# rasmusab/bayes.js

Hardware: AMD Instinct MI355X
Metric: posterior draws/sec (= param-updates/sec) (higher is better)
Workload: dtype f64

## Files before the change

bayes.js_amd/csrc/amwg_kernel.h:

```cpp
#pragma once
#if !defined(__HIPCC_RTC__)
#include <hip/hip_runtime.h>
#endif

#include "amwg_div.h"
#include "amwg_ld.h"
#include "amwg_philox.h"
#include "amwg_types.h"

namespace amwg {

struct LdsLayout {
  uint32_t data, state, pls, cnt, tot, cc, adapt, pl, idx, perm, total, stride, logpls, bc, xw;
};
__host__ __device__ inline LdsLayout lds_layout(size_t data_bytes, int P, int CPB, int max_top, int n_named, bool multi = false) {
  LdsLayout L;
  uint32_t o = 0;
  L.stride = (uint32_t)P | 1u;
  L.data = o;  o += (uint32_t)((data_bytes + 15) & ~(size_t)15);
  L.state = o; o += L.stride * CPB * 8;
  L.pls = o;   o += L.stride * CPB * 8;
  L.cnt = o;   o += L.stride * CPB * 8;
  L.tot = o;   o += (L.stride * CPB * 4 + 15) & ~15u;
  L.cc = o;    o += (uint32_t)P * sizeof(CompConst);
  L.adapt = o; o += ((uint32_t)P + 7) & ~7u;
  L.pl = o;    o += (uint32_t)n_named * 20u;
  o = (o + 15) & ~15u;
  L.idx = o;   o += (max_top > 1) ? (((uint32_t)max_top * CPB * (max_top > kByteTop ? 2u : 1u) + 15) & ~15u) : 0;
  L.perm = o;  o += (n_named > kPackedNamed) ? (((uint32_t)n_named * CPB * 2u + 15) & ~15u) : 0;
  L.logpls = o; o += multi ? L.stride * CPB * 8 : 0;
  L.bc = o;     o += multi ? ((L.stride * CPB * 4 + 15) & ~15u) : 0;
  L.xw = o;     o += multi ? 2u * 16u * 8u : 0;
  L.total = (o + 15) & ~15u;
  return L;
}

template <class Model, bool FAST, int G, int U = Model::kUnroll>
__device__ __forceinline__ double pass_over_data(const typename Model::Pass &ps, int n_obs, int sub, double acc) {
  const int n_full = n_obs / G, rem = n_obs % G;
  int k = 0;
  for (; k + U <= n_full; k += U) {
    double t[U];
#pragma unroll
    for (int u = 0; u < U; ++u) t[u] = Model::template term<FAST>(ps, (k + u) * G + sub);
#pragma unroll
    for (int u = 0; u < U; ++u) acc += t[u];
  }
  for (; k < n_full; ++k) acc += Model::template term<FAST>(ps, k * G + sub);
  if (sub < rem) acc += Model::template term<FAST>(ps, n_full * G + sub);
  return acc;
}

struct CrossWave {
  double *buf;
  int parity;
};

template <class...> using void_of = void;

template <class M, class = void> struct BinaryOf { static constexpr bool value = true; };
template <class M> struct BinaryOf<M, void_of<decltype(M::kHasBinary)>> { static constexpr bool value = M::kHasBinary; };

template <class M, class = void> struct TracksState { static constexpr bool value = false; };
template <class M> struct TracksState<M, void_of<decltype(M::kTracksState)>> { static constexpr bool value = M::kTracksState; };

template <class M, class = void> struct LaneReuseOf { static constexpr bool value = false; };
template <class M> struct LaneReuseOf<M, void_of<decltype(M::kLaneReuse)>> { static constexpr bool value = M::kLaneReuse; };

template <class M, class = void> struct CertifiedOf { static constexpr bool value = false; static constexpr int lanes = 0; };
template <class M> struct CertifiedOf<M, void_of<decltype(M::kCertified)>> { static constexpr bool value = M::kCertified; static constexpr int lanes = M::kCertifiedLanes; };
template <class M, int G, class = void> struct CertifiedAt { static constexpr bool value = false; };
template <class M, int G> struct CertifiedAt<M, G, void_of<decltype(M::kCertified)>> { static constexpr bool value = M::kCertified && M::kCertifiedLanes == G; };

template <class M, class = void> struct CertNeedsRows { static constexpr bool value = false; };
template <class M> struct CertNeedsRows<M, void_of<decltype(M::kCertifiedNeedsRows)>> { static constexpr bool value = M::kCertifiedNeedsRows; };

template <class M, class = void> struct RefOrderOf { static constexpr bool value = false; };
template <class M> struct RefOrderOf<M, void_of<decltype(M::kReferenceOrder)>> { static constexpr bool value = M::kReferenceOrder; };

template <class M, class = void> struct OwnPassOf { static constexpr bool value = false; };
template <class M> struct OwnPassOf<M, void_of<decltype(M::kOwnPass)>> { static constexpr bool value = M::kOwnPass; };

struct NoCache {};
template <class M, class = void> struct CacheOf { using type = NoCache; static __device__ __forceinline__ type init() { return type{}; } };
template <class M> struct CacheOf<M, void_of<typename M::Cache>> { using type = typename M::Cache; static __device__ __forceinline__ type init() { return M::cache_init(); } };

template <int OFF, bool EXACT = false>
__device__ __forceinline__ double xor_partner(double v) {
#if defined(__HIP_DEVICE_COMPILE__)
  int lo = (int)(uint32_t)f64_bits(v), hi = (int)(uint32_t)(f64_bits(v) >> 32);
  if constexpr (OFF == 1) {
    lo = __builtin_amdgcn_mov_dpp(lo, 0xB1, 0xF, 0xF, true); hi = __builtin_amdgcn_mov_dpp(hi, 0xB1, 0xF, 0xF, true);
  } else if constexpr (OFF == 2) {
    lo = __builtin_amdgcn_mov_dpp(lo, 0x4E, 0xF, 0xF, true); hi = __builtin_amdgcn_mov_dpp(hi, 0x4E, 0xF, 0xF, true);
  } else if constexpr (OFF == 4) {
    lo = __builtin_amdgcn_mov_dpp(lo, 0x141, 0xF, 0xF, true); hi = __builtin_amdgcn_mov_dpp(hi, 0x141, 0xF, 0xF, true);
    if constexpr (EXACT) {
      lo = __builtin_amdgcn_mov_dpp(lo, 0x1B, 0xF, 0xF, true); hi = __builtin_amdgcn_mov_dpp(hi, 0x1B, 0xF, 0xF, true);
    }
  } else if constexpr (OFF == 8) {
    lo = __builtin_amdgcn_mov_dpp(lo, 0x140, 0xF, 0xF, true); hi = __builtin_amdgcn_mov_dpp(hi, 0x140, 0xF, 0xF, true);
    if constexpr (EXACT) {
      lo = __builtin_amdgcn_mov_dpp(lo, 0x141, 0xF, 0xF, true); hi = __builtin_amdgcn_mov_dpp(hi, 0x141, 0xF, 0xF, true);
    }
  } else if constexpr (OFF == 16) {
    lo = __builtin_amdgcn_ds_swizzle(lo, 0x401F); hi = __builtin_amdgcn_ds_swizzle(hi, 0x401F);
  } else {
    return __shfl_xor(v, OFF, 64);
  }
  return bits_f64(((uint64_t)(uint32_t)hi << 32) | (uint64_t)(uint32_t)lo);
#else
  return v;
#endif
}
template <int OFF, bool EXACT = false>
__device__ __forceinline__ double xor_sum(double acc) {
#if defined(__HIP_DEVICE_COMPILE__)
  if constexpr (OFF == 16 || OFF == 32) {
    const uint32_t lo = (uint32_t)f64_bits(acc), hi = (uint32_t)(f64_bits(acc) >> 32);
    if constexpr (OFF == 32) {
      const auto l = __builtin_amdgcn_permlane32_swap(lo, lo, false, false), h = __builtin_amdgcn_permlane32_swap(hi, hi, false, false);
      return bits_f64(((uint64_t)h[0] << 32) | (uint64_t)l[0]) + bits_f64(((uint64_t)h[1] << 32) | (uint64_t)l[1]);
    } else {
      const auto l = __builtin_amdgcn_permlane16_swap(lo, lo, false, false), h = __builtin_amdgcn_permlane16_swap(hi, hi, false, false);
      return bits_f64(((uint64_t)h[0] << 32) | (uint64_t)l[0]) + bits_f64(((uint64_t)h[1] << 32) | (uint64_t)l[1]);
    }
  } else {
    return acc + xor_partner<OFF, EXACT>(acc);
  }
#else
  return acc;
#endif
}
template <int OFF, int LIMIT>
__device__ __forceinline__ double butterfly(double acc) {
  if constexpr (OFF < LIMIT) { acc = xor_sum<OFF>(acc); return butterfly<OFF * 2, LIMIT>(acc); }
  else return acc;
}

#ifndef AMWG_STEPPER_PRIORITY
#define AMWG_STEPPER_PRIORITY 2
#endif
constexpr int kStepperPriority = AMWG_STEPPER_PRIORITY;
__device__ __forceinline__ void wave_priority(int p) {
#if defined(__HIP_DEVICE_COMPILE__)
  if (kStepperPriority > 0) { if (p == 0) __builtin_amdgcn_s_setprio(0); else __builtin_amdgcn_s_setprio(kStepperPriority); }
#endif
}

__device__ __forceinline__ int fresh_uniform(int v) {
#if defined(__HIP_DEVICE_COMPILE__)
#if !defined(AMWG_X_NOFRESH)
  v = __builtin_amdgcn_readfirstlane(v);
  asm volatile("" : "+s"(v));
#endif
#endif
  return v;
}

template <class Model, int G, int U = 8>
__device__ __forceinline__ double log_post(const StateView &S, const StepArgs &a0, const unsigned char *smem, int sub, CrossWave &xw,
// ... 285 lines not shown
#else
  return v;
#endif
}

constexpr int kErrReplicasNeedOneWave = 1, kErrLaunchTooLong = 2, kErrMirrorOutOfSync = 4, kErrSweepNeedsOrderInRegisters = 8, kErrNoKernelBody = 16;
__device__ __forceinline__ void device_error(const StepArgs &a, int code) {
#if defined(__HIP_DEVICE_COMPILE__)
  if (threadIdx.x == 0) (void)atomicOr(a.ch.error, code);
#endif
}
template <class M, class = void> struct MirrorCheckOf { static constexpr bool value = false; };
template <class M> struct MirrorCheckOf<M, void_of<decltype(M::kMirrorCheck)>> { static constexpr bool value = M::kMirrorCheck; };

template <class Model, int G, int BT = 256, bool GL = false, bool SW = false, bool CT = false>
__device__ __forceinline__ void step_body(const StepArgs &a, unsigned char *smem) {
  constexpr int kPassU = SW ? (CertNeedsRows<Model>::value ? 2 : 4) : (BT >= 1024 ? 4 : 8);
  const int tid = threadIdx.x, nt = blockDim.x;
  constexpr bool kMulti = G > 64;
  if (!kMulti && a.cpb > 0 && nt != 64) { device_error(a, kErrReplicasNeedOneWave); return; }
  if (a.n_steps > 65535) { device_error(a, kErrLaunchTooLong); return; }
  const int CPB = kMulti ? G / 64 : ((a.cpb > 0 && a.cpb < nt / G) ? a.cpb : nt / G);
  const int c_raw = kMulti ? tid / 64 : tid / G;
  const int c_in = c_raw < CPB ? c_raw : CPB - 1, sub = tid % G;
  const int P = a.pl.P;
  const int n_named = a.pl.n_params;
  const LdsLayout L = lds_layout(DataBytesOf<Model, GL>::get(a.d, G, nt), P, CPB, a.pl.max_top, n_named, kMulti);

  const unsigned char *data_lds = smem + L.data;
  double *Sblk = reinterpret_cast<double *>(smem + L.state);
  CompConst *cc = reinterpret_cast<CompConst *>(smem + L.cc);
  uint8_t *adapt = smem + L.adapt;
  int32_t *pl_base = reinterpret_cast<int32_t *>(smem + L.pl), *pl_len = pl_base + n_named, *pl_top = pl_len + n_named, *pl_multidim = pl_top + n_named, *pl_inner = pl_multidim + n_named;
  const bool wide_idx = a.pl.max_top > kByteTop, wide_perm = n_named > kPackedNamed;
  const IndexColumn idx{smem + L.idx + (wide_idx ? 2 * c_in : c_in), CPB, wide_idx};
  const IndexColumn pcol{smem + L.perm + 2 * c_in, CPB, true};
  double *SDme = reinterpret_cast<double *>(smem + L.pls) + (size_t)c_in * L.stride;
  int2 *CNTme = reinterpret_cast<int2 *>(smem + L.cnt) + (size_t)c_in * L.stride;
  uint32_t *TOTme = reinterpret_cast<uint32_t *>(smem + L.tot) + (size_t)c_in * L.stride;
  double *LOGPLSme = reinterpret_cast<double *>(smem + L.logpls) + (size_t)c_in * L.stride;
  int32_t *BCme = reinterpret_cast<int32_t *>(smem + L.bc) + (size_t)c_in * L.stride;
  CrossWave xw{reinterpret_cast<double *>(smem + L.xw), 0};
  typename CacheOf<Model>::type cache = CacheOf<Model>::init();

  Model::stage(smem + L.data, a.d, tid, nt, G);
  for (int p = tid; p < P; p += nt) { cc[p] = a.cc[p]; adapt[p] = a.is_adapting[p]; }
  for (int i = tid; i < 4 * n_named; i += nt) pl_base[i] = a.pl.tab[i];
  for (int i = tid; i < n_named; i += nt) pl_inner[i] = a.pl.tab[n_named + i] / a.pl.tab[2 * n_named + i];

  const int64_t chain_raw = kMulti ? (int64_t)blockIdx.x : (int64_t)blockIdx.x * CPB + c_in;
  const bool live = chain_raw < a.C;
  const int64_t cl = live ? chain_raw : a.C - 1;
  const bool writer = live && sub == 0;
  const bool counter = sub == 0 && c_raw < CPB;
  const int64_t C = a.C;

  double *Sme = Sblk + (size_t)c_in * L.stride;
  for (int p = 0; p < P; ++p) {
    Sme[p] = a.ch.state[p * C + cl];
    SDme[p] = exp_v8(a.ch.prop_log_scale[p * C + cl]);
    CNTme[p] = make_int2(a.ch.acceptance_count[p * C + cl], a.ch.iterations_since_adaption[p * C + cl]);
    TOTme[p] = 0u;
    if constexpr (kMulti) { LOGPLSme[p] = a.ch.prop_log_scale[p * C + cl]; BCme[p] = a.ch.batch_count[p * C + cl]; }
  }
  const StateView S{Sme};
  uint64_t perm = wide_perm ? 0ull : a.ch.perm[cl];
  if (wide_perm)
    for (int k = 0; k < n_named; ++k) pcol.set(k, (int)a.ch.perm16[(int64_t)k * C + cl]);
  typename RngOf<Model, G, GL, SW>::type rng;
  if constexpr (GL) rng.init(a.seed, a.chain_offset + (uint64_t)cl, a.ch.rng_n[cl], tid, reinterpret_cast<double *>(smem + L.data + Model::gl_lds_bytes(a.d.pad, 0)) + (size_t)(tid >> 6) * 256);
  else if constexpr (SW) rng.init(a.seed, a.chain_offset + (uint64_t)cl, a.ch.rng_n[cl], tid, reinterpret_cast<double *>(smem + L.data + Model::window_offset(a.d, nt / 64)) + (size_t)(tid >> 6) * 256);
  else rng.init(a.seed, a.chain_offset + (uint64_t)cl, a.ch.rng_n[cl], tid);
  double lp_curr = a.ch.lp_curr[cl];
  __syncthreads();
  constexpr bool kCert = CT && CertifiedAt<Model, G>::value && !GL && (SW == CertNeedsRows<Model>::value);
  static_assert(kCert == CT, "a certified kernel is instantiated for a model that has no certified value at this lane count");
  constexpr bool kRefOrder = kCert && G > 1 && RefOrderOf<Model>::value;
  auto expression = [&]() -> double {
    if constexpr (kRefOrder) return Model::template reference_order<G>(cache, S, a.mc, a.d, data_lds, sub);
    else if constexpr (!GL) return log_post<Model, G, kPassU>(S, a, data_lds, sub, xw, cache);
    else return 0.0;
  };
  if constexpr (!GL) { if (a.init_lp) lp_curr = expression(); }
  double lpA = lp_curr, epsA = 0.0;
  bool lp_exact = true;
  if constexpr (kCert) { if (!a.init_lp) { epsA = a.ch.lp_eps[cl]; lp_exact = epsA == 0.0; } }
  (void)lpA; (void)epsA; (void)lp_exact;
#if defined(AMWG_AUDIT)
  constexpr bool kAudit = kCert;
#else
  constexpr bool kAudit = false;
#endif
  [[maybe_unused]] double audE = 0.0, aud_max_v = 0.0, aud_max_d = 0.0;
  [[maybe_unused]] uint32_t aud_n = 0u, aud_bad = 0u;
  [[maybe_unused]] auto audit_bin = [&](int which, double ratio) {
#if defined(AMWG_AUDIT)
    if (writer) {
      int b = 0;
      if (ratio > 0.0) { b = (int)((f64_bits(ratio) >> 52) & 0x7ffu) - 1023 + 40; b = b < 1 ? 1 : (b > 63 ? 63 : b); }
      if (!(ratio == ratio)) b = 63;
      (void)atomicAdd(cold_args()->ch.audit_hist + which * 64 + b, 1ull);
    }
#endif
  };
  [[maybe_unused]] auto audit_adversarial_u = [&](double ex, double eta, double u, int parity) -> double {
    if (!(eta < 0x1p-8) || !(ex > 0x1p-900) || !(ex < kInf)) return u;
    const double below = ex * (1.0 - 1.5 * eta), above = ex * (1.0 + 1.5 * eta);
    const double v = ((parity & 1) && above < 1.0) ? above : below;
    return (v > 0.0 && v < 1.0) ? v : u;
  };
  [[maybe_unused]] auto audit_value = [&](double A, double eps, double E) {
    if (eps == eps && eps < kInf && eps > 0.0 && E == E && __builtin_fabs(E) < kInf) {
      const double r = __builtin_fabs(A - E) / eps;
      aud_max_v = (r > aud_max_v || !(r == r)) ? r : aud_max_v;
      audit_bin(0, r);
    }
  };
  [[maybe_unused]] auto audit_difference = [&](double dA, double eta0, double dE, int verdict, double u) {
    if (eta0 == eta0 && eta0 < kInf && eta0 > 0.0 && dE == dE && __builtin_fabs(dE) < kInf) {
      const double r = __builtin_fabs(dA - dE) / eta0;
      aud_max_d = (r > aud_max_d || !(r == r)) ? r : aud_max_d;
      audit_bin(1, r);
    }
    const bool exact_acc = exp_v8(dE) > u;
    ++aud_n;
    if ((verdict > 0 && !exact_acc) || (verdict < 0 && exact_acc)) ++aud_bad;
  };
#if defined(AMWG_X_PHASES)
  uint64_t ph_acc[16];
#pragma unroll
  for (int q = 0; q < 16; ++q) ph_acc[q] = 0;
  uint64_t ph_last = __builtin_readcyclecounter();
#define AMWG_PHASE(i) do { const uint64_t ph_now = __builtin_readcyclecounter(); ph_acc[i] += ph_now - ph_last; ph_last = ph_now; } while (0)
#else
#define AMWG_PHASE(i) do { } while (0)
#endif
  auto set_state = [&](int comp, double v) {
    Sme[comp] = v;
    if constexpr (TracksState<Model>::value) Model::on_set(cache, comp, v, sub, a.d);
  };

  constexpr int D = Model::kDerived;
  const int PR = P + D;
  int64_t row = a.row0;
  int32_t next_rec = (int32_t)a.step0;
  const int P_stepped = a.pl.P_stepped;
  const bool recording = a.draws != nullptr;
  const int n_steps = a.n_steps;

  const int lane64 = tid & 63;
  int ord = lane64;
  (void)ord;
  if (SW && a.pl.max_top > 64) { device_error(a, kErrSweepNeedsOrderInRegisters); return; }
  const bool ord_in_regs = SW ? true : (G >= 64 && a.pl.max_top <= 64);
  constexpr bool kSweep = SW && !GL && LaneReuseOf<Model>::value && G == 64 && !BinaryOf<Model>::value;
  const bool sweep_rt = kSweep && ord_in_regs && a.d.pad > 0;
  if constexpr (kAudit) { if (lp_exact) audE = lp_curr; else audE = expression(); }
  wave_priority(kStepperPriority);
  auto record_draws = [&](int step) {
    if (recording && step == next_rec) {
      double *const draws = cold_args()->draws;
      {
        constexpr int LW = G < 64 ? G : 64;
        if (live && (!kMulti || sub < 64))
          for (int p = sub & (LW - 1); p < P; p += LW) {
#if !defined(AMWG_X_NOREC)
            draws[(row * PR + p) * C + cl] = S(p);
#endif
          }
      }
      if constexpr (D > 0) {
        double dv[D];
        (void)Model::template eval<G, true>(S, a.d, data_lds, sub, dv);
        if (writer)
          for (int q = 0; q < D; ++q) draws[(row * PR + P + q) * C + cl] = dv[q];
      }
      ++row;
      next_rec += cold_args()->thin;
    }
  };
  auto shuffle_named = [&]() {
    for (int i = n_named - 1; i > 0; --i) {
      const int j = (int)__builtin_floor(rng.next() * (double)(i + 1));
      if (wide_perm) { const int ti = pcol.get(i); pcol.set(i, pcol.get(j)); pcol.set(j, ti); }
      else perm = perm_swap(perm, i, j);
    }
  };
  auto adapt_component = [&](int comp, bool accepted, int2 cnt, double batch_size, bool store, bool per_lane = false) {
    cnt.x += accepted ? 1 : 0;
    cnt.y += 1;
    const bool boundary = (double)cnt.y >= batch_size;
    if (per_lane ? boundary : chain_true<GL ? 1 : G>(boundary)) {
      const CompConst k = cc[comp];
      const int64_t gi = (int64_t)comp * C + cl;
      int32_t *const g_bc = kMulti ? nullptr : cold_args()->ch.batch_count;
      double *const g_pls = kMulti ? nullptr : cold_args()->ch.prop_log_scale;
      const int32_t bc = (kMulti ? BCme[comp] : g_bc[gi]) + 1;
      const double adj = __builtin_fmin(k.max_adaptation, k.initial_adaptation / __builtin_sqrt((double)bc));
      double pls = kMulti ? LOGPLSme[comp] : g_pls[gi];
      if ((double)cnt.x / k.batch_size > k.target_accept_rate) pls += adj; else pls -= adj;
      cnt = make_int2(0, 0);
      SDme[comp] = exp_v8_cold(pls);
      if constexpr (kMulti) { BCme[comp] = bc; LOGPLSme[comp] = pls; }
      else if (store) { g_bc[gi] = bc; g_pls[gi] = pls; }
    }
    CNTme[comp] = cnt;
  };

  [[maybe_unused]] auto accept_sweep = [&](double diff, double u_accept) -> bool {
    bool accepted = false;
    if (chain_true<G>(diff >= 0.0)) accepted = true;
    else if (chain_true<G>(diff < -746.0)) accepted = false;
    else {
      const double lower = 1.0 + diff;
      if (chain_true<G>(u_accept < lower - 0x1p-50)) accepted = true;
// ... 429 lines not shown
              const double Tv = rows.comp == c ? rows.T_new : T_cur;
              const double prop_lp = butterfly<1, 64>(Tv);
              if (accept_sweep(prop_lp - lp_curr, u_c)) { lp_curr = prop_lp; T_cur = Tv; set_state(sb + c, prop_c); acc_mask |= 1ull << c; }
            }
            if (lane64 < d_len) {
              const bool inb_l = ((inb_s >> lane64) & 1ull) != 0ull, acc_l = ((acc_mask >> lane64) & 1ull) != 0ull;
              if (inb_l) TOTme[sb + lane64] += 1u + (acc_l ? 0x10000u : 0u);
              if (adapt[sb + lane64] != 0) adapt_component(sb + lane64, acc_l, CNTme[sb + lane64], cc[sb + lane64].batch_size, live, true);
            }
            Model::sweep_done(cache, rows, rows.comp >= 0 && ((acc_mask >> (rows.comp & 63)) & 1ull) != 0ull);
            if constexpr (kCert) { lpA = lp_curr; epsA = 0.0; }
            e = 0; e_top = 0; e_in = 0; ++np;
            slot += d_len - 1;
            if (slot + 1 < P_stepped) nx = prefetch(next_comp());
            continue;
          }
          sw_left = d_len;
          }
#endif
        }
      }
      const SlotPre me = nx;
      const int comp = me.comp;
      const double k_lower = cc[comp].lower, k_upper = cc[comp].upper;
      const int k_type = cc[comp].type;
      if (BinaryOf<Model>::value && k_type == kTypeBinary) {
        const double old = me.cur;
        set_state(comp, 0.0);
        const double zero_ld = log_post<Model, G, kPassU>(S, a, data_lds, sub, xw, cache);
        set_state(comp, 1.0);
        const double one_ld = log_post<Model, G, kPassU>(S, a, data_lds, sub, xw, cache);
        const double mx = js_max2(zero_ld, one_ld);
        const double z = zero_ld - mx, o = one_ld - mx;
        const double zero_prob = exp_v8(z - log_v8(exp_v8(z) + exp_v8(o)));
        double now = 1.0;
        lp_curr = one_ld;
        if (rng.next() < zero_prob) { set_state(comp, 0.0); now = 0.0; lp_curr = zero_ld; }
        if (counter) (void)__hip_atomic_fetch_add(&TOTme[comp], 1u + ((now != old) ? 0x10000u : 0u), __ATOMIC_RELAXED, __HIP_MEMORY_SCOPE_WORKGROUP);
        if (slot + 1 < P_stepped) nx = prefetch(next_comp());
        continue;
      }
      AMWG_PHASE(14);
      const double cur = me.cur;
      const bool in_sweep = kSweep && sw_left > 0;
      double prop;
      if (in_sweep) prop = lane_value(sw_prop, comp - sb);
      else {
        prop = rnorm_js(rng, cur, me.sd);
        if (chain_true<G>(k_type == kTypeInt)) prop = js_round(prop);
      }
      const bool inb = chain_true<G>(!(prop < k_lower || prop > k_upper));
      double u_accept = 0.0;
      if (inb) { set_state(comp, prop); u_accept = in_sweep ? lane_value(sw_u, comp - sb) : rng.next(); }
      if (in_sweep) --sw_left;
      AMWG_PHASE(8);
      if (slot + 1 < P_stepped) nx = prefetch(next_comp());
      AMWG_PHASE(9);
      bool accepted = false;
      bool certified = false;
      [[maybe_unused]] double aud_E_prop = 0.0;
      if constexpr (kCert) {
        if (__ballot(inb) != 0ull) {
          wave_priority(0);
          const typename Model::Approx r = Model::template log_post_approx<G, BT>(cache, S, a.mc, a.d, data_lds, sub);
          wave_priority(kStepperPriority);
          AMWG_PHASE(10);
          if (inb) {
            const double dA = r.value - lpA;
            const double eta = ((r.eps + epsA + __builtin_fabs(dA) * 0x1p-51) * 1.0625 + 0x1p-49) * a.bound_scale;
            const double ex = exp_v8(dA);
            if constexpr (kAudit) { if (a.audit_adversarial) u_accept = audit_adversarial_u(ex, eta, u_accept, step + slot); }
            const int verdict = certified_test(dA, eta, ex, u_accept);
            if constexpr (kAudit) {
              aud_E_prop = expression();
              audit_value(r.value, r.eps, aud_E_prop);
              audit_difference(dA, (r.eps + epsA + __builtin_fabs(dA) * 0x1p-51) * 1.0625, aud_E_prop - audE, verdict, u_accept);
            }
            if (chain_true<G>(verdict > 0)) { certified = true; accepted = true; lpA = r.value; epsA = r.eps; lp_exact = false; }
            else if (chain_true<G>(verdict < 0)) { certified = true; set_state(comp, cur); }
            if (certified && counter) (void)__hip_atomic_fetch_add(&TOTme[comp], 1u + (accepted ? 0x10000u : 0u), __ATOMIC_RELAXED, __HIP_MEMORY_SCOPE_WORKGROUP);
          }
        }
      }
      if (certified) {
      } else if (inb) {
        double prop_lp = 0.0;
        if constexpr (kCert) {
          for (int which = chain_true<G>(lp_exact) ? 1 : 0; which < 2; ++which) {
            if (which == 0) set_state(comp, cur);
            const double v = expression();
            if (which == 0) { lp_curr = v; lp_exact = true; set_state(comp, prop); }
            else prop_lp = v;
          }
        } else {
          prop_lp = expression();
        }
#if defined(__HIP_DEVICE_COMPILE__)
        asm volatile("" : : "v"(nx.cur), "v"(nx.sd), "v"(nx.batch_size), "v"(nx.cnt.x), "v"(nx.cnt.y), "v"((int)nx.adapting));
#endif
        const double diff = prop_lp - lp_curr;
        if (chain_true<G>(diff >= 0.0)) accepted = true;
        else if (chain_true<G>(diff < -746.0)) accepted = false;
        else {
          const double lower = 1.0 + diff;
          if (chain_true<G>(u_accept < lower - 0x1p-50)) accepted = true;
          else if (chain_true<G>(diff > -1.0 && u_accept > (lower + 0.5 * diff * diff) + 0x1p-50)) accepted = false;
          else accepted = chain_true<G>(exp_v8(diff) > u_accept);
        }
        accepted = chain_true<G>(accepted);
        if (accepted) lp_curr = prop_lp;
        else set_state(comp, cur);
        if constexpr (kCert) { lpA = lp_curr; epsA = 0.0; }
        if (counter) (void)__hip_atomic_fetch_add(&TOTme[comp], 1u + (accepted ? 0x10000u : 0u), __ATOMIC_RELAXED, __HIP_MEMORY_SCOPE_WORKGROUP);
      }
      if constexpr (kAudit) { if (inb && accepted) audE = aud_E_prop; }
      AMWG_PHASE(11);
      if (chain_true<G>(me.adapting)) adapt_component(comp, accepted, me.cnt, me.batch_size, writer);
      AMWG_PHASE(12);
    }
  }

  if constexpr (kCert) {
    if (a.finalize_lp && !lp_exact) { lp_curr = expression(); lp_exact = true; }
    if (!lp_exact) lp_curr = lpA;
    if (writer) cold_args()->ch.lp_eps[cl] = lp_exact ? 0.0 : epsA;
  }
  if constexpr (!GL && MirrorCheckOf<Model>::value) {
    if (!Model::template mirror_ok<G>(cache, S, a.d, sub)) (void)atomicOr(cold_args()->ch.error, kErrMirrorOutOfSync);
  }
#if defined(AMWG_X_PHASES)
  if ((tid & 63) == 0 && live) {
    unsigned long long *const hh = cold_args()->ch.audit_hist + 64;
#pragma unroll
    for (int q = 0; q < 16; ++q) (void)atomicAdd(hh + q, (unsigned long long)ph_acc[q]);
  }
#endif
  if constexpr (kAudit) {
    if (writer) {
      double *const au = cold_args()->ch.audit;
      const double v0 = au[cl], d0 = au[C + cl];
      au[cl] = (aud_max_v > v0 || !(aud_max_v == aud_max_v)) ? aud_max_v : v0;
      au[C + cl] = (aud_max_d > d0 || !(aud_max_d == aud_max_d)) ? aud_max_d : d0;
      au[2 * C + cl] += (double)aud_n;
      au[3 * C + cl] += (double)aud_bad;
    }
  }
  if (writer) {
    const cold_args_ptr ca = cold_args();
    double *const o_state = ca->ch.state, *const o_pls = ca->ch.prop_log_scale;
    int32_t *const o_ac = ca->ch.acceptance_count, *const o_it = ca->ch.iterations_since_adaption, *const o_bc = ca->ch.batch_count;
    int32_t *const o_acc = ca->ch.accepts, *const o_inb = ca->ch.inbounds;
    for (int p = 0; p < P; ++p) {
      o_state[p * C + cl] = S(p);
      o_ac[p * C + cl] = CNTme[p].x;
      o_it[p * C + cl] = CNTme[p].y;
      o_acc[p * C + cl] += (int32_t)(TOTme[p] >> 16);
      o_inb[p * C + cl] += (int32_t)(TOTme[p] & 0xffffu);
      if constexpr (kMulti) { o_pls[p * C + cl] = LOGPLSme[p]; o_bc[p * C + cl] = BCme[p]; }
    }
    if (wide_perm) { uint16_t *const o_p16 = ca->ch.perm16; for (int k = 0; k < n_named; ++k) o_p16[(int64_t)k * C + cl] = (uint16_t)pcol.get(k); }
    else ca->ch.perm[cl] = perm;
    ca->ch.rng_n[cl] = rng.consumed();
    ca->ch.lp_curr[cl] = lp_curr;
  }
}

template <class M, class = void> struct MinWavesOf { static constexpr int value = 1; };
template <class M> struct MinWavesOf<M, void_of<decltype(M::kMinWavesPerSimd)>> { static constexpr int value = M::kMinWavesPerSimd; };

template <class Model, int G, int BT>
__global__ void __launch_bounds__(BT, MinWavesOf<Model>::value) amwg_step_kernel(const StepArgs a) {
  extern __shared__ __attribute__((aligned(16))) unsigned char smem[];
  step_body<Model, G, BT>(a, smem);
}
template <class Model, int BT>
__global__ void __launch_bounds__(BT, MinWavesOf<Model>::value) amwg_sweep_kernel(const StepArgs a) {
  extern __shared__ __attribute__((aligned(16))) unsigned char smem[];
  step_body<Model, 64, BT, false, true>(a, smem);
}
template <class Model, int G, int BT>
__global__ void __launch_bounds__(BT, MinWavesOf<Model>::value) amwg_step_kernel_cert(const StepArgs a) {
  extern __shared__ __attribute__((aligned(16))) unsigned char smem[];
  step_body<Model, G, BT, false, false, true>(a, smem);
}
template <class Model, int BT>
__global__ void __launch_bounds__(BT, MinWavesOf<Model>::value) amwg_sweep_kernel_cert(const StepArgs a) {
  extern __shared__ __attribute__((aligned(16))) unsigned char smem[];
  step_body<Model, 64, BT, false, true, true>(a, smem);
}
template <class Model, int BT>
__global__ void __launch_bounds__(BT, MinWavesOf<Model>::value) amwg_gl_kernel(const StepArgs a) {
  extern __shared__ __attribute__((aligned(16))) unsigned char smem[];
  step_body<Model, 64, BT, true>(a, smem);
}

}
```

bayes.js_amd/csrc/amwg_models.h:

```cpp
#pragma once
#include "amwg_div.h"
#include "amwg_ld.h"
#include "amwg_pass.h"
#include "amwg_twoval.h"
#include "amwg_types.h"
#include "amwg_window.h"

namespace amwg {

__device__ __forceinline__ double norm_const_sd(double v, double m, double c_sd, double den, double y_hi, double y_lo, int den_ok) {
  const double t = v - m;
  const double tt = t * t;
  const double q = (den_ok && wide_range(tt)) ? div_by_invariant(tt, den, Reciprocal{y_hi, y_lo}) : tt / den;
  return c_sd - q;
}

struct NormCache {
  double sd, c, den;
  Reciprocal y;
  bool den_ok;
};
__device__ __forceinline__ NormCache norm_cache_init() { return NormCache{__builtin_nan(""), 0.0, 0.0, Reciprocal{0.0, 0.0}, false}; }
AMWG_HD NormCache norm_cache_make(double sd, double neg_half_log_2pi) {
  NormCache k;
// ... 42 lines not shown
    for (int i = tid; i < d.n_obs; i += nt) dst[i] = d.x[i];
  }
  template <class C>
  __device__ __forceinline__ static double prior(const StateView &, const ModelConsts &mc, const DataRef &, C &kc) {
    double lp = 0;
    lp += norm_const_sd(kc.mu, mc.m0, mc.c0, mc.den0, mc.y0_hi, mc.y0_lo, mc.den0_ok);
    const double sigma = kc.sigma;
    lp += (sigma < mc.ua || sigma > mc.ub) ? -kInf : mc.lunif;
    return lp;
  }
  static constexpr bool kTracksState = true;
  struct Cache { NormCache n; double mu, sigma; bool loaded; };
  __device__ __forceinline__ static Cache cache_init() { return Cache{norm_cache_init(), 0.0, 0.0, false}; }
  __device__ __forceinline__ static void on_set(Cache &k, int comp, double v, int, const DataRef &) { k.mu = comp == 0 ? v : k.mu; k.sigma = comp == 0 ? k.sigma : v; }
  static constexpr bool kMirrorCheck = true;
  template <int GL>
  __device__ __forceinline__ static bool mirror_ok(const Cache &k, const StateView &S, const DataRef &, int) {
    return !k.loaded || (f64_bits(k.mu) == f64_bits(S(0)) && f64_bits(k.sigma) == f64_bits(S(1)));
  }
  template <int GL>
  __device__ __forceinline__ static void load(Cache &k, const StateView &S, const ModelConsts &, const DataRef &, const unsigned char *, int) {
    if (!k.loaded) { k.mu = S(0); k.sigma = S(1); k.loaded = true; }
  }
  template <int GL>
  __device__ __forceinline__ static Pass begin(const StateView &, const ModelConsts &mc, const DataRef &d,
                                               const unsigned char *smem, Cache &kc) {
    Pass ps;
    NormCache &k = kc.n;
    ps.mu = kc.mu;
    norm_cache_update(k, kc.sigma, mc.neg_half_log_2pi);
    ps.c = k.c;
    ps.den = k.den;
    ps.y = k.y;
    ps.fast = !mc.exact_division && mc.data_mid_range && k.den_ok &&
              (ps.mu == 0 || mid_range(__builtin_fabs(ps.mu)));
    ps.x = GL == 1 ? d.x : reinterpret_cast<const double *>(smem);
    return ps;
  }
  template <bool FAST>
  __device__ __forceinline__ static double term(const Pass &ps, int i) {
    const double t = ps.x[i] - ps.mu;
    const double tt = t * t;
    return ps.c - (FAST ? div_by_invariant(tt, ps.den, ps.y) : tt / ps.den);
  }
  template <int G>
  __device__ inline __attribute__((noinline)) static double pass_slow_impl(const double *x, double mu, double c, double den, int n_obs, int sub, double acc) {
    for (int i = sub; i < n_obs; i += G) { const double t = x[i] - mu; acc += c - (t * t) / den; }
    return acc;
  }
  template <int G>
  __device__ __forceinline__ static double pass_slow(const Pass &ps, int n_obs, int sub, double acc) { return pass_slow_impl<G>(ps.x, ps.mu, ps.c, ps.den, n_obs, sub, acc); }
  static constexpr bool kStagedFast = true;
  template <int G, int U = 8>
  __device__ __forceinline__ static double pass_fast(const Pass &ps, int n_obs, int sub, double acc) {
    if constexpr (G == 1) return norm_pass_uniform<8>(ps.x, ps.mu, ps.c, ps.den, ps.y, n_obs, acc);
    else return norm_pass_staged<G, U, false>(ps.x, nullptr, StateView{nullptr}, ps.mu, ps.c, ps.den, ps.y, n_obs, sub, acc);
  }
  static constexpr bool kCertified = true;
  static constexpr int kCertifiedLanes = 1;
  struct Approx { double value, eps; };
  template <int G, int BT>
  __device__ __forceinline__ static Approx log_post_approx(Cache &kc, const StateView &S, const ModelConsts &mc, const DataRef &d, const unsigned char *smem, int sub) {
    static_assert(G == 1, "the certified pass of the Normal family is the one-lane one");
    load<G>(kc, S, mc, d, smem, sub);
    norm_cache_update(kc.n, kc.sigma, mc.neg_half_log_2pi);
    const double P = prior(S, mc, d, kc);
    double S2;
    if (mc.sufficient) {
      const double dm = (mc.suff_xbar_hi - kc.mu) + mc.suff_xbar_lo;
      S2 = __builtin_fma((double)d.n_obs, dm * dm, mc.suff_ss);
    } else
    if constexpr (BT <= 512) {
      constexpr int B = BT <= 256 ? kWaveBlock : 8;
      double *scr = wave_scratch_of(d);
      const bool tile = lds_bytes_of(d, 1, 0) != 0;
      if (tile && scr != nullptr) S2 = norm_sq_pass_wave<B, true>((amwg_lds_f64_ptr)smem, kc.mu, d.n_obs, scr);
      else S2 = norm_sq_pass_wave<B>(tile ? reinterpret_cast<const double *>(smem) : d.x, kc.mu, d.n_obs, scr);
    }
    else S2 = norm_sq_pass_uniform<8>(d.x, kc.mu, d.n_obs);
    const double n = (double)d.n_obs;
    const double Q = S2 * kc.n.y.hi, nc = n * kc.n.c;
    const double mag = __builtin_fabs(P) + __builtin_fabs(nc) + 2.0 * Q;
    return Approx{(P + nc) - Q, (2.0 * n + 64.0) * 0x1p-53 * mag * 1.25};
  }
};

struct BetaBernModel {
  static constexpr bool kSplitPrior = false;
  static constexpr bool kUser = false, kHasFast = false, kOneLanePass = true;
  static constexpr int kDerived = 0;
  static constexpr bool kHasBinary = false;
  static constexpr int kMaxThreads = 1024;
  static constexpr int kUnroll = 8;
  struct Pass { double l1, l0; const uint8_t *x; const uint32_t *bits; bool has_invalid, fast_forward; BitData B; };
  __host__ __device__ static size_t words(int n_obs) { return (size_t)n_obs / 32 + 2; }
  static constexpr size_t kFfLdsLimit = 120 * 1024;
  __host__ __device__ static size_t lds_bytes(int n_obs, int, int lanes) {
    if (lanes == 1) { const size_t b = 6 * words(n_obs) * 4; return b <= kFfLdsLimit ? ((b + 15) & ~(size_t)15) : 0; }
    return ((size_t)n_obs + 15) & ~(size_t)15;
  }
  __device__ static void stage(unsigned char *smem, const DataRef &d, int tid, int nt, int lanes) {
    if (lanes == 1) {
      if (lds_bytes(d.n_obs, 0, 1) == 0) return;
      uint32_t *dst = reinterpret_cast<uint32_t *>(smem);
      const uint32_t *src = static_cast<const uint32_t *>(d.arr[0]);
      for (int k = tid; k < (int)(6 * words(d.n_obs)); k += nt) dst[k] = src[k];
      return;
    }
    for (int i = tid; i < d.n_obs; i += nt) smem[i] = d.xb[i];
  }
  template <class C>
  __device__ __forceinline__ static double prior(const StateView &S, const ModelConsts &mc, const DataRef &, C &) {
    const double th = S(0);
    double lp = 0;
    if (th > 1 || th < 0) lp += -kInf;
    else if (mc.ba == 1 && mc.bb == 1) lp += 0.0;
    else lp += (mc.ba - 1) * log_v8(th) + (mc.bb - 1) * log_v8(1 - th) - mc.lbeta_ab;
    return lp;
  }
  struct Cache {};
  __device__ __forceinline__ static Cache cache_init() { return Cache{}; }
  template <int GL>
  __device__ __forceinline__ static Pass begin(const StateView &S, const ModelConsts &mc, const DataRef &d,
                                               const unsigned char *smem, Cache &) {
    Pass ps;
    const double th = S(0);
    ps.l1 = log_v8(th);
    ps.l0 = log_v8(1 - th);
    ps.x = smem;
    ps.bits = d.xw;
    ps.has_invalid = mc.has_invalid != 0;
    ps.fast_forward = !mc.exact_division;
    {
      const size_t W = words(d.n_obs);
      const uint32_t *base = lds_bytes(d.n_obs, 0, 1) ? reinterpret_cast<const uint32_t *>(smem) : static_cast<const uint32_t *>(d.arr[0]);
      ps.B.w = base; ps.B.pre = base + W; ps.B.om1 = base + 2 * W; ps.B.po1 = base + 3 * W; ps.B.om0 = base + 4 * W; ps.B.po0 = base + 5 * W;
      ps.B.n = d.n_obs;
    }
    return ps;
  }
  template <bool FAST>
  __device__ __forceinline__ static double term(const Pass &ps, int i) { return ps.x[i] ? ps.l1 : ps.l0; }

#define AMWG_A0 "v_add_f64 %[acc], %[acc], %[l0]\n"
#define AMWG_A1 "v_add_f64 %[acc], %[acc], %[l1]\n"
#define AMWG_N0 AMWG_A0 AMWG_A0 AMWG_A0 AMWG_A0
#define AMWG_N1 AMWG_A1 AMWG_A0 AMWG_A0 AMWG_A0
#define AMWG_N2 AMWG_A0 AMWG_A1 AMWG_A0 AMWG_A0
#define AMWG_N3 AMWG_A1 AMWG_A1 AMWG_A0 AMWG_A0
#define AMWG_N4 AMWG_A0 AMWG_A0 AMWG_A1 AMWG_A0
#define AMWG_N5 AMWG_A1 AMWG_A0 AMWG_A1 AMWG_A0
#define AMWG_N6 AMWG_A0 AMWG_A1 AMWG_A1 AMWG_A0
#define AMWG_N7 AMWG_A1 AMWG_A1 AMWG_A1 AMWG_A0
#define AMWG_N8 AMWG_A0 AMWG_A0 AMWG_A0 AMWG_A1
#define AMWG_N9 AMWG_A1 AMWG_A0 AMWG_A0 AMWG_A1
#define AMWG_N10 AMWG_A0 AMWG_A1 AMWG_A0 AMWG_A1
#define AMWG_N11 AMWG_A1 AMWG_A1 AMWG_A0 AMWG_A1
#define AMWG_N12 AMWG_A0 AMWG_A0 AMWG_A1 AMWG_A1
#define AMWG_N13 AMWG_A1 AMWG_A0 AMWG_A1 AMWG_A1
#define AMWG_N14 AMWG_A0 AMWG_A1 AMWG_A1 AMWG_A1
#define AMWG_N15 AMWG_A1 AMWG_A1 AMWG_A1 AMWG_A1
#define AMWG_B(HI, LO) AMWG_N##LO AMWG_N##HI "s_branch 25b\n"
#define AMWG_ROW(HI)                                                                                   \
  AMWG_B(HI, 0) AMWG_B(HI, 1) AMWG_B(HI, 2) AMWG_B(HI, 3) AMWG_B(HI, 4) AMWG_B(HI, 5) AMWG_B(HI, 6) AMWG_B(HI, 7) \
  AMWG_B(HI, 8) AMWG_B(HI, 9) AMWG_B(HI, 10) AMWG_B(HI, 11) AMWG_B(HI, 12) AMWG_B(HI, 13) AMWG_B(HI, 14) AMWG_B(HI, 15)
#define AMWG_BERN_ADD_BIT0                                                                             \
// ... 800 lines not shown
```

Before: 1.475 billion.

## Evaluate uncertified exact log-posteriors cooperatively across the wave for normal model

When only a few lanes in a wave fail the certified approximate accept test, the wave now computes their exact log-posteriors together. Each observation row is split across lanes and summed serially with readlane, in place of each lane running its own full serial pass while the other lanes idle. It handles the current and proposed states together when both are needed, and is capped by a small maximum number of lanes. It also adds phase-timing counters under a debug flag. The risk is extra readlane overhead and a larger kernel when many lanes need the fallback.

```diff
diff --git a/bayes.js_amd/csrc/amwg_kernel.h b/bayes.js_amd/csrc/amwg_kernel.h
--- a/bayes.js_amd/csrc/amwg_kernel.h
+++ b/bayes.js_amd/csrc/amwg_kernel.h
@@ -77,6 +77,9 @@
 
 template <class M, class = void> struct RefOrderOf { static constexpr bool value = false; };
 template <class M> struct RefOrderOf<M, void_of<decltype(M::kReferenceOrder)>> { static constexpr bool value = M::kReferenceOrder; };
+
+template <class M, int G, class = void> struct WaveExactAt { static constexpr bool value = false; };
+template <class M, int G> struct WaveExactAt<M, G, void_of<decltype(M::kWaveExactLanes)>> { static constexpr bool value = M::kWaveExactLanes == G; };
 
 template <class M, class = void> struct OwnPassOf { static constexpr bool value = false; };
 template <class M> struct OwnPassOf<M, void_of<decltype(M::kOwnPass)>> { static constexpr bool value = M::kOwnPass; };
@@ -528,6 +531,7 @@
     else return 0.0;
   };
   if constexpr (!GL) { if (a.init_lp) lp_curr = expression(); }
+  constexpr bool kWaveExact = kCert && WaveExactAt<Model, G>::value;
   double lpA = lp_curr, epsA = 0.0;
   bool lp_exact = true;
   if constexpr (kCert) { if (!a.init_lp) { epsA = a.ch.lp_eps[cl]; lp_exact = epsA == 0.0; } }
@@ -577,6 +581,8 @@
 #pragma unroll
   for (int q = 0; q < 16; ++q) ph_acc[q] = 0;
   uint64_t ph_last = __builtin_readcyclecounter();
+  const uint64_t ph_born = ph_last;
+  uint32_t ph_exact_slots = 0u, ph_exact_evals = 0u;
 #define AMWG_PHASE(i) do { const uint64_t ph_now = __builtin_readcyclecounter(); ph_acc[i] += ph_now - ph_last; ph_last = ph_now; } while (0)
 #else
 #define AMWG_PHASE(i) do { } while (0)
@@ -1172,10 +1178,29 @@
           }
         }
       }
+#if defined(AMWG_X_PHASES)
+      if constexpr (kCert) {
+        const uint64_t ph_fb = __ballot(inb && !certified);
+        if (ph_fb != 0ull) { ++ph_exact_slots; ph_exact_evals += (uint32_t)(__builtin_popcountll(ph_fb) + __builtin_popcountll(__ballot(inb && !certified && !lp_exact))); }
+      }
+#endif
+      double prop_lp = 0.0;
+      [[maybe_unused]] bool exact_done = false;
+      if constexpr (kWaveExact) {
+        const bool need = inb && !certified;
+        const uint64_t need_mask = __ballot(need);
+        if (need_mask != 0ull && __builtin_popcountll(need_mask) <= Model::kWaveExactMax) {
+          const bool both = need && !lp_exact;
+          const typename Model::Exact2 ex2 = Model::template exact_wave<G>(cache, S, a.mc, a.d, data_lds, comp, cur, need_mask, __ballot(both));
+          if (both) { lp_curr = ex2.cur; lp_exact = true; }
+          if (need) prop_lp = ex2.prop;
+          exact_done = true;
+        }
+      }
       if (certified) {
       } else if (inb) {
-        double prop_lp = 0.0;
         if constexpr (kCert) {
+          if (!exact_done)
           for (int which = chain_true<G>(lp_exact) ? 1 : 0; which < 2; ++which) {
             if (which == 0) set_state(comp, cur);
             const double v = expression();
@@ -1223,6 +1248,11 @@
     unsigned long long *const hh = cold_args()->ch.audit_hist + 64;
 #pragma unroll
     for (int q = 0; q < 16; ++q) (void)atomicAdd(hh + q, (unsigned long long)ph_acc[q]);
+    const unsigned long long life = (unsigned long long)(__builtin_readcyclecounter() - ph_born);
+    (void)atomicAdd(hh + 16, life);                                      (void)atomicMax(hh + 17, life);
+    (void)atomicAdd(hh + 18, (unsigned long long)ph_exact_slots);        (void)atomicMax(hh + 19, (unsigned long long)ph_exact_slots);
+    (void)atomicAdd(hh + 20, (unsigned long long)ph_exact_evals);        (void)atomicMax(hh + 21, (unsigned long long)ph_exact_evals);
+    (void)atomicAdd(hh + 22, 1ull);
   }
 #endif
   if constexpr (kAudit) {
diff --git a/bayes.js_amd/csrc/amwg_models.h b/bayes.js_amd/csrc/amwg_models.h
--- a/bayes.js_amd/csrc/amwg_models.h
+++ b/bayes.js_amd/csrc/amwg_models.h
@@ -148,6 +148,109 @@
     const double Q = S2 * kc.n.y.hi, nc = n * kc.n.c;
     const double mag = __builtin_fabs(P) + __builtin_fabs(nc) + 2.0 * Q;
     return Approx{(P + nc) - Q, (2.0 * n + 64.0) * 0x1p-53 * mag * 1.25};
+  }
+
+  static constexpr int kWaveExactLanes = 1;
+#ifndef AMWG_WAVE_EXACT_MAX
+#define AMWG_WAVE_EXACT_MAX 2
+#endif
+  static constexpr int kWaveExactMax = AMWG_WAVE_EXACT_MAX;
+  struct Exact2 { double cur, prop; };
+  template <int NS>
+  __device__ __forceinline__ static void exact_wave_rows(const double *x, int n_obs, int lane, const double (&mu)[NS], const double (&sg)[NS], double nhl2pi, int fast_ok, double (&acc)[NS]) {
+#if defined(__HIP_DEVICE_COMPILE__)
+    NormCache k[NS];
+    bool fast[NS];
+#pragma unroll
+    for (int s = 0; s < NS; ++s) {
+      k[s] = norm_cache_make(sg[s], nhl2pi);
+      const bool f = fast_ok != 0 && k[s].den_ok && (mu[s] == 0 || mid_range(__builtin_fabs(mu[s])));
+      fast[s] = __builtin_amdgcn_readfirstlane((int)f) != 0;
+    }
+    const int n_full = n_obs >> 6, rem = n_obs & 63, n_rows = n_full + (rem != 0 ? 1 : 0);
+    if (n_rows == 0) return;
+    const int last = n_obs - 1;
+    double xn = x[lane < last ? lane : last];
+    for (int r = 0; r < n_rows; ++r) {
+      const double xv = xn;
+      const int inext = 64 * (r + 1) + lane;
+      xn = x[inext < last ? inext : last];
+      double term[NS];
+#pragma unroll
+      for (int s = 0; s < NS; ++s) {
+        const double t = xv - mu[s];
+        const double tt = t * t;
+        term[s] = k[s].c - (fast[s] ? div_by_invariant(tt, k[s].den, k[s].y) : tt / k[s].den);
+      }
+      if (r < n_full) {
+        constexpr int B = NS == 1 ? 32 : 16;
+#pragma unroll
+        for (int b = 0; b < 64; b += B) {
+          double v[NS][B];
+#pragma unroll
+          for (int l = 0; l < B; ++l)
+#pragma unroll
+            for (int s = 0; s < NS; ++s) v[s][l] = lane_value_of(term[s], b + l);
+#pragma unroll
+          for (int l = 0; l < B; ++l)
+#pragma unroll
+            for (int s = 0; s < NS; ++s) acc[s] += v[s][l];
+        }
+      } else {
+        for (int l = 0; l < rem; ++l)
+#pragma unroll
+          for (int s = 0; s < NS; ++s) acc[s] += lane_value_of(term[s], l);
+      }
+    }
+#endif
+  }
+  __device__ __forceinline__ static double lane_value_of(double v, int src) {
+#if defined(__HIP_DEVICE_COMPILE__)
+    const uint32_t hi = (uint32_t)__builtin_amdgcn_readlane((int)(f64_bits(v) >> 32), src);
+    const uint32_t lo = (uint32_t)__builtin_amdgcn_readlane((int)(uint32_t)f64_bits(v), src);
+    return bits_f64(((uint64_t)hi << 32) | (uint64_t)lo);
+#else
+    return v;
+#endif
+  }
+  __device__ inline __attribute__((noinline)) static Exact2 exact_wave_sum(uint64_t need, uint64_t both, double mu_c, double sg_c, double pr_c, double mu_p, double sg_p, double pr_p,
+                                                                           double nhl2pi, int fast_ok, const double *x, int n_obs) {
+    Exact2 out{0.0, 0.0};
+#if defined(__HIP_DEVICE_COMPILE__)
+    const int lane = (int)__builtin_amdgcn_mbcnt_hi(~0u, __builtin_amdgcn_mbcnt_lo(~0u, 0u));
+    uint32_t need_lo = (uint32_t)__builtin_amdgcn_readfirstlane((int)(uint32_t)need), need_hi = (uint32_t)__builtin_amdgcn_readfirstlane((int)(uint32_t)(need >> 32));
+    const uint32_t both_lo = (uint32_t)__builtin_amdgcn_readfirstlane((int)(uint32_t)both), both_hi = (uint32_t)__builtin_amdgcn_readfirstlane((int)(uint32_t)(both >> 32));
+    uint64_t todo = ((uint64_t)need_hi << 32) | need_lo;
+    const uint64_t two_of = ((uint64_t)both_hi << 32) | both_lo;
+    n_obs = __builtin_amdgcn_readfirstlane(n_obs);
+    while (todo != 0ull) {
+      const int src = (int)__builtin_ctzll(todo);
+      todo &= todo - 1ull;
+      if ((two_of >> src) & 1ull) {
+        const double mu[2] = {lane_value_of(mu_c, src), lane_value_of(mu_p, src)}, sg[2] = {lane_value_of(sg_c, src), lane_value_of(sg_p, src)};
+        double acc[2] = {lane_value_of(pr_c, src), lane_value_of(pr_p, src)};
+        exact_wave_rows<2>(x, n_obs, lane, mu, sg, nhl2pi, fast_ok, acc);
+        if (lane == src) { out.cur = acc[0]; out.prop = acc[1]; }
+      } else {
+        const double mu[1] = {lane_value_of(mu_p, src)}, sg[1] = {lane_value_of(sg_p, src)};
+        double acc[1] = {lane_value_of(pr_p, src)};
+        exact_wave_rows<1>(x, n_obs, lane, mu, sg, nhl2pi, fast_ok, acc);
+        if (lane == src) out.prop = acc[0];
+      }
+    }
+#endif
+    return out;
+  }
+  template <int G>
+  __device__ __forceinline__ static Exact2 exact_wave(Cache &kc, const StateView &S, const ModelConsts &mc, const DataRef &d, const unsigned char *smem, int comp, double cur,
+                                                      uint64_t need, uint64_t both) {
+    static_assert(G == 1, "a lane per chain");
+    load<G>(kc, S, mc, d, smem, 0);
+    struct MuSigma { double mu, sigma; };
+    MuSigma p{kc.mu, kc.sigma}, c{comp == 0 ? cur : kc.mu, comp == 0 ? kc.sigma : cur};
+    const double pr_p = prior(S, mc, d, p), pr_c = prior(S, mc, d, c);
+    const double *x = lds_bytes_of(d, 1, 0) != 0 ? reinterpret_cast<const double *>(smem) : d.x;
+    return exact_wave_sum(need, both, c.mu, c.sigma, pr_c, p.mu, p.sigma, pr_p, mc.neg_half_log_2pi, (!mc.exact_division && mc.data_mid_range) ? 1 : 0, x, d.n_obs);
   }
 };
 
```

Result: no change. 1.484 billion (median of 6 runs) (+0.6%).
